# googlegenomics/spark-examples

Measured on NVIDIA H100. Metric: genotype-cells/sec (N x V) into Gram, higher is better.
Workload: dtype int8

## Files before the change

spark_examples_b200/csrc/gram_sm90.cu:

```cuda
#include <cuda.h>
#include <cuda_runtime.h>

#include <cstring>

#include <algorithm>
#include <map>
#include <mutex>
#include <tuple>
#include <type_traits>
#include <cstdio>
#include <cstdlib>
#include <string>
#include <vector>

#include "ptx_sm90.cuh"
#include "vpca_internal.h"

namespace vpca {

namespace {

constexpr int kThreads = 384;
constexpr int kKBytes = 128;
constexpr int kBoxRows = 128;
// ... 331 lines not shown
        const int cnt = kbw < kb_end - base ? kbw : kb_end - base;
        s.kb0 = base + (plan.lo[i] < cnt ? plan.lo[i] : cnt);
        s.kb1 = base + (plan.hi[i] < cnt ? plan.hi[i] : cnt);
        s.win = win;
        s.last_in_win = (seg_i == plan.n);
        s.col = plan.col[i];
        s.slot = i;
        s.first = (win == 0);
        s.flush = (win == nwin - 1);
        s.use = 0;
        return true;
    }
};

__device__ __forceinline__ void mbar_wait(uint32_t bar, uint32_t parity, int* err, int code) {
    if (ptx::mbar_try_wait(bar, parity)) return;
    const long long t0 = clock64();
    while (!ptx::mbar_try_wait(bar, parity)) {
        if (clock64() - t0 > kWatchdogCycles) {
            if (err != nullptr) {
                err[0] = code;
                err[1] = (int)blockIdx.x;
                err[2] = (int)bar;
                err[3] = (int)parity;
                __threadfence_system();
            }
            __trap();
        }
    }
}

__device__ __forceinline__ long long globaltimer_ns() {
    long long t;
    asm volatile("mov.u64 %0, %%globaltimer;" : "=l"(t));
    return t;
}

__device__ __forceinline__ void wait_window(const int* win_done, int w, int need) {
    const long long t0 = globaltimer_ns();
    while (true) {
        int v;
        asm volatile("ld.acquire.gpu.global.s32 %0, [%1];" : "=r"(v) : "l"(win_done + w) : "memory");
        if (v >= need) return;
        if (globaltimer_ns() - t0 > 200000) return;
        __nanosleep(256);
    }
}

__device__ __forceinline__ uint64_t make_smem_desc(uint32_t saddr) {
    return (uint64_t)((saddr & 0x3FFFFu) >> 4) | (1ull << 16) | ((uint64_t)(1024 >> 4) << 32) | (1ull << 62);
}

__device__ __forceinline__ uint32_t e2m1x4_to_s8x2(uint32_t w) {
    const uint32_t mag = __byte_perm(0x03020100u, 0x0C080604u, w & 0x7777u);
    const uint32_t sgn = ((w >> 3) & 1u) | (((w >> 7) & 1u) << 8) | (((w >> 11) & 1u) << 16) | (((w >> 15) & 1u) << 24);
    const uint32_t m = sgn * 0xFFu;
    return (mag & ~m) | (__vneg4(mag) & m);
}

__device__ __forceinline__ int quarter_rn(int acc) {
    const int q = acc >> 2, r = acc & 3;
    return q + ((r > 2 || (r == 2 && (q & 1))) ? 1 : 0);
}

template <int KIND>
using AccT = typename std::conditional<KIND == 1, float, uint32_t>::type;

template <int KIND>
__device__ __forceinline__ int acc_to_int(AccT<KIND> v) {
    if constexpr (KIND == 0) return (int)v;
    else if constexpr (KIND == 1) return __float2int_rn(v);
    else return quarter_rn((int)v);
}

template <int CG, int KIND>
__global__ void __launch_bounds__(kThreads, 1) gram_kernel(const __grid_constant__ CUtensorMap tmap, const GramArgs a) {
    using C = Cfg<KIND>;
    extern __shared__ uint8_t smem_raw[];
    const uint32_t smem_base = (ptx::smem_u32(smem_raw) + 1023u) & ~1023u;
    const uint32_t bar_base = smem_base + C::STAGES * C::STAGE_BYTES + C::XBUF_BYTES * 2;
    auto sB = [&](uint32_t st) { return smem_base + st * C::STAGE_BYTES; };
    auto sA = [&](uint32_t st) { return smem_base + st * C::STAGE_BYTES + C::B_BYTES; };
    auto full_bar = [&](uint32_t i) { return bar_base + 8u * i; };
    auto empty_bar = [&](uint32_t i) { return bar_base + 8u * (C::STAGES + i); };

    const int warp = __shfl_sync(0xffffffffu, (int)(threadIdx.x >> 5), 0);
    const uint32_t lane = ptx::lane_id();
    const uint32_t cta_rank = (CG == 2) ? (blockIdx.x & 1u) : 0u;
    const int worker = (CG == 2) ? (int)(blockIdx.x >> 1) : (int)blockIdx.x;
    auto release = [&](uint32_t st) {
        if constexpr (CG == 2) {
            ptx::mbar_arrive_cluster(ptx::mapa(empty_bar(st), 0));
            ptx::mbar_arrive_cluster(ptx::mapa(empty_bar(st), 1));
        } else {
            ptx::mbar_arrive(empty_bar(st));
        }
    };

    if (warp == 0 && ptx::elect_one()) {
        ptx::prefetch_tensormap(&tmap);
        for (uint32_t i = 0; i < (uint32_t)C::STAGES; ++i) {
            ptx::mbar_init(full_bar(i), 1);
            ptx::mbar_init(empty_bar(i), 2 * CG);
        }
        ptx::fence_mbar_init();
    }
    if constexpr (CG == 2) ptx::cluster_sync();
    else __syncthreads();
    if (a.prof != nullptr && threadIdx.x == 0) a.prof[(size_t)blockIdx.x * 4 + 0] = globaltimer_ns();

    if (warp < 4) {
        asm volatile("setmaxnreg.dec.sync.aligned.u32 40;");
        if (warp == 0 && ptx::elect_one()) {
            const bool leader = cta_rank == 0;
            Sched sc;
            sc.init(a, worker);
            Seg s;
            uint32_t it = 0;
            int synced_win = -1;
            while (sc.next(s)) {
                const int rowA = (CG == 2 && cta_rank != 0) ? s.rowA1 : s.rowA0;
                const bool two_boxes = s.n_eff > kBoxRows;
                const bool self_b = (CG == 2) && (s.flags & kTileSelfB) != 0;
                const uint32_t tx = (uint32_t)((two_boxes ? 2 : 1) + (self_b ? 0 : 1)) * C::BOX_BYTES;
                if (a.sync_lead > 0 && leader && s.win != synced_win) {
                    synced_win = s.win;
                    if (s.win >= a.sync_lead) wait_window(a.win_done, s.win - a.sync_lead, a.active_workers);
                }
                for (int kb = s.kb0; kb < s.kb1; ++kb, ++it) {
                    const uint32_t st = it % C::STAGES, ph = (it / C::STAGES) & 1u;
                    mbar_wait(empty_bar(st), ph ^ 1u, a.err, 1);
                    const int pnl = kb / a.kb_per_panel;
                    const int kc = (kb - pnl * a.kb_per_panel) * a.kc_per_kb;
                    ptx::mbar_arrive_expect_tx(full_bar(st), tx);
                    if constexpr (CG == 2) {
                        if (two_boxes || cta_rank == 0)
                            ptx::tma_load_3d_multicast(sB(st) + cta_rank * C::BOX_BYTES, &tmap, full_bar(st), kc,
                                                       s.rowB + (int)cta_rank * kBoxRows, pnl, 0x3);
                    } else {
                        ptx::tma_load_3d(sB(st), &tmap, full_bar(st), kc, s.rowB, pnl);
                        if (two_boxes) ptx::tma_load_3d(sB(st) + C::BOX_BYTES, &tmap, full_bar(st), kc, s.rowB + kBoxRows, pnl);
                    }
                    if (!self_b) ptx::tma_load_3d(sA(st), &tmap, full_bar(st), kc, rowA, pnl);
                }
                if (a.sync_lead > 0 && leader && s.last_in_win)
                    asm volatile("red.release.gpu.global.add.s32 [%0], 1;" ::"l"(a.win_done + s.win) : "memory");
            }
        }
    } else {
        asm volatile("setmaxnreg.inc.sync.aligned.u32 232;");
        const int cw = (warp >> 2) - 1;
        const int wq = warp & 3;
        const uint32_t ctid = threadIdx.x - 128;
        AccT<KIND> acc[2][64];
        Sched sc;
        sc.init(a, worker);
        Seg s;
        uint32_t it = 0;
        while (sc.next(s)) {
            const bool filler = (CG == 2) && cta_rank != 0 && (s.flags & kTileFiller) != 0;
            const bool self_b = (CG == 2) && (s.flags & kTileSelfB) != 0;
            const int mrow0 = cw * 128;
            const bool act0 = mrow0 < s.n_eff, act1 = mrow0 + 64 < s.n_eff;
            if (s.first) {
#pragma unroll
                for (int i = 0; i < 64; ++i) {
                    acc[0][i] = 0;
                    acc[1][i] = 0;
                }
            }
            const uint32_t a_off = (self_b ? cta_rank : 2u) * (uint32_t)(kBoxRows * 128);
            int pending = -1;
            for (int kb = s.kb0; kb < s.kb1; ++kb, ++it) {
                const uint32_t st = it % C::STAGES, ph = (it / C::STAGES) & 1u;
                mbar_wait(full_bar(st), ph, a.err, 3);
                uint32_t opB, opA;
                if constexpr (KIND == 2) {
                    const uint32_t xb = smem_base + C::STAGES * C::STAGE_BYTES + (it & 1u) * C::XBUF_BYTES;
                    ptx::named_sync(1, 256);
                    const int nb = s.n_eff > kBoxRows ? 2 * kBoxRows : kBoxRows;
                    const int rows = nb + (self_b ? 0 : kBoxRows);
                    for (int c = (int)ctid; c < rows * 8; c += 256) {
                        const int r = c >> 3, j = c & 7;
                        const uint32_t src = (r < nb ? sB(st) + (uint32_t)r * 64u : sA(st) + (uint32_t)(r - nb) * 64u) + (uint32_t)j * 8u;
                        const int xr = r < nb ? r : 2 * kBoxRows + (r - nb);
                        uint32_t lo, hi;
                        asm volatile("ld.shared.v2.u32 {%0, %1}, [%2];" : "=r"(lo), "=r"(hi) : "r"(src));
                        const uint32_t o0 = e2m1x4_to_s8x2(lo & 0xFFFFu), o1 = e2m1x4_to_s8x2(lo >> 16);
                        const uint32_t o2 = e2m1x4_to_s8x2(hi & 0xFFFFu), o3 = e2m1x4_to_s8x2(hi >> 16);
                        const uint32_t dst = xb + (uint32_t)xr * 128u + (((uint32_t)j ^ ((uint32_t)xr & 7u)) << 4);
                        asm volatile("st.shared.v4.u32 [%0], {%1, %2, %3, %4};" ::"r"(dst), "r"(o0), "r"(o1), "r"(o2), "r"(o3)
                                     : "memory");
                    }
                    ptx::fence_proxy_async();
                    ptx::named_sync(1, 256);
                    if (threadIdx.x % 128 == 0) release(st);
                    opB = xb;
                } else {
                    opB = sB(st);
                }
                opA = opB + a_off;
                const uint64_t bdesc = make_smem_desc(opA);
                const uint64_t adesc0 = make_smem_desc(opB + (uint32_t)mrow0 * 128u);
                const uint64_t adesc1 = make_smem_desc(opB + (uint32_t)(mrow0 + 64) * 128u);
                ptx::wgmma_fence_acc(acc[0]);
                ptx::wgmma_fence_acc(acc[1]);
                ptx::wgmma_fence();
#pragma unroll
                for (int k = 0; k < kKBytes / 32; ++k) {
                    if constexpr (KIND == 1) {
                        ptx::wgmma_bf16(acc[0], adesc0 + 2 * k, bdesc + 2 * k);
                        ptx::wgmma_bf16(acc[1], adesc1 + 2 * k, bdesc + 2 * k);
                    } else {
                        ptx::wgmma_s8(acc[0], adesc0 + 2 * k, bdesc + 2 * k);
                        ptx::wgmma_s8(acc[1], adesc1 + 2 * k, bdesc + 2 * k);
                    }
                }
                ptx::wgmma_commit();
                ptx::wgmma_wait<1>();
                ptx::wgmma_fence_acc(acc[0]);
                ptx::wgmma_fence_acc(acc[1]);
                if constexpr (KIND != 2) {
                    if (pending >= 0 && threadIdx.x % 128 == 0) release((uint32_t)pending);
                }
                pending = (int)st;
            }
            ptx::wgmma_wait<0>();
            ptx::wgmma_fence_acc(acc[0]);
            ptx::wgmma_fence_acc(acc[1]);
            if constexpr (KIND != 2) {
                if (pending >= 0 && threadIdx.x % 128 == 0) release((uint32_t)pending);
            }
            if (!s.flush || filler) continue;

            const int colA = (CG == 2 && cta_rank != 0) ? s.rowA1 : s.rowA0;
            const int row_end = min(a.row_limit, s.rowB + s.n_eff);
            const bool pair64 = a.red64 != 0 && (a.n & 1) == 0;
#pragma unroll
            for (int j = 0; j < 2; ++j) {
                if (!(j == 0 ? act0 : act1)) continue;
#pragma unroll
                for (int h = 0; h < 2; ++h) {
                    const int row = s.rowB + mrow0 + 64 * j + 16 * wq + (int)(lane >> 2) + 8 * h;
                    if (row >= row_end) continue;
                    int32_t* own = a.S;
                    if (a.num_peers != 0 && a.peer_mode == 1) {
                        int o = 0;
                        while (o + 1 < a.num_peers && row >= a.own_end[o]) ++o;
                        own = a.peer[o];
                    }
#pragma unroll
                    for (int i = 0; i < 16; ++i) {
                        const int col = colA + 8 * i + 2 * (int)(lane & 3);
                        if (col >= a.n) continue;
                        int v0 = acc_to_int<KIND>(acc[j][4 * i + 2 * h]);
                        int v1 = acc_to_int<KIND>(acc[j][4 * i + 2 * h + 1]);
                        if ((s.flags & kTileXpose) != 0 && (row >> 7) < (col >> 7)) {
                            for (int e = 0; e < 2; ++e) {
                                const int v = e ? v1 : v0, c = col + e;
                                if (v == 0 || c >= a.n) continue;
                                const size_t o = (size_t)c * (size_t)a.n + (size_t)row;
                                if (a.num_peers == 0) {
                                    asm volatile("red.global.add.s32 [%0], %1;" ::"l"(a.S + o), "r"(v) : "memory");
                                } else if (a.peer_mode == 1) {
                                    int q = 0;
                                    while (q + 1 < a.num_peers && c >= a.own_end[q]) ++q;
                                    asm volatile("red.relaxed.sys.global.add.s32 [%0], %1;" ::"l"(a.peer[q] + o), "r"(v) : "memory");
                                } else {
                                    for (int d = 0; d < a.num_peers; ++d)
                                        asm volatile("red.relaxed.sys.global.add.s32 [%0], %1;" ::"l"(a.peer[d] + o), "r"(v)
                                                     : "memory");
                                }
                            }
                            continue;
                        }
                        if (row < col) v0 = 0;
                        if (row < col + 1 || col + 1 >= a.n) v1 = 0;
                        if ((v0 | v1) == 0) continue;
                        const size_t o = (size_t)row * (size_t)a.n + (size_t)col;
                        if (pair64) {
                            const unsigned long long packed = (unsigned long long)(unsigned)v0 | ((unsigned long long)(unsigned)v1 << 32);
                            if (a.num_peers == 0) {
                                asm volatile("red.global.add.u64 [%0], %1;" ::"l"(a.S + o), "l"(packed) : "memory");
                            } else if (a.peer_mode == 1) {
                                asm volatile("red.relaxed.sys.global.add.u64 [%0], %1;" ::"l"(own + o), "l"(packed) : "memory");
                            } else {
                                for (int d = 0; d < a.num_peers; ++d)
                                    asm volatile("red.relaxed.sys.global.add.u64 [%0], %1;" ::"l"(a.peer[d] + o), "l"(packed)
                                                 : "memory");
                            }
                        } else {
                            for (int e = 0; e < 2; ++e) {
                                const int v = e ? v1 : v0;
                                if (v == 0) continue;
                                if (a.num_peers == 0) {
                                    asm volatile("red.global.add.s32 [%0], %1;" ::"l"(a.S + o + e), "r"(v) : "memory");
                                } else if (a.peer_mode == 1) {
                                    asm volatile("red.relaxed.sys.global.add.s32 [%0], %1;" ::"l"(own + o + e), "r"(v) : "memory");
                                } else {
                                    for (int d = 0; d < a.num_peers; ++d)
                                        asm volatile("red.relaxed.sys.global.add.s32 [%0], %1;" ::"l"(a.peer[d] + o + e), "r"(v)
                                                     : "memory");
                                }
                            }
                        }
                    }
                }
            }
        }
        if (a.prof != nullptr && threadIdx.x == 128) a.prof[(size_t)blockIdx.x * 4 + 2] = globaltimer_ns();
    }

    if constexpr (CG == 2) ptx::cluster_sync();
    else __syncthreads();
    if (a.prof != nullptr && threadIdx.x == 0) a.prof[(size_t)blockIdx.x * 4 + 3] = globaltimer_ns();
}

__global__ void rebalance_kernel(const long long* __restrict__ prof, double* __restrict__ cum, int workers, int cta_group,
                                 double gain, double max_share, long long min_ns, int* __restrict__ gen, const TileDesc* __restrict__ tiles,
                                 int num_tiles, int total_weight, int kbw, int col_limit) {
    __shared__ double sh[1024];
    __shared__ double cand[1025];
    __shared__ long long need[1025];
    __shared__ double red_sum, red_min;
    __shared__ int reject, need_repair;
    const int w = threadIdx.x;
    const bool active = w < workers;
    double t = 0.0, share_old = 0.0;
    if (active) {
        const long long t0 = prof[(size_t)w * cta_group * 4 + 0], t1 = prof[(size_t)w * cta_group * 4 + 2];
        t = (double)(t1 - t0);
        share_old = cum[w + 1] - cum[w];
    }
    sh[w] = active ? t : 1e30;
    if (w == 0) {
        reject = 0;
        need_repair = 0;
    }
    __syncthreads();
    if (w == 0) {
        double mn = 1e30, mx = 0.0;
        for (int i = 0; i < workers; ++i) {
            mn = fmin(mn, sh[i]);
            mx = fmax(mx, sh[i]);
        }
        red_min = (mn < (double)min_ns || (mx - mn) < 0.03 * mx) ? -1.0 : mn;
    }
    __syncthreads();
    if (red_min < 0.0) return;
    const double speed = active ? share_old / t : 0.0;
    sh[w] = speed;
    __syncthreads();
    if (w == 0) {
        double sum = 0.0;
        for (int i = 0; i < workers; ++i) sum += sh[i];
        red_sum = sum;
    }
    __syncthreads();
    double share = 0.0;
    if (active) {
        const double est = speed / red_sum;
        share = (1.0 - gain) * share_old + gain * est;
        const double avg = 1.0 / workers;
        share = fmin(fmax(share, 0.5 * avg), max_share * avg);
    }
    __syncthreads();
    sh[w] = share;
    __syncthreads();
    if (w == 0) {
        double sum = 0.0;
        for (int i = 0; i < workers; ++i) sum += sh[i];
        double acc = 0.0;
        cand[0] = 0.0;
        for (int i = 0; i < workers; ++i) {
            acc += sh[i] / sum;
            cand[i + 1] = (i + 1 == workers) ? 1.0 : acc;
        }
    }
    __syncthreads();
    if (active) {
        const long long uw = (long long)total_weight * kbw;
        const long long ub = (long long)((double)uw * cand[w]);
        const long long ue = (w + 1 == workers) ? uw : (long long)((double)uw * cand[w + 1]);
        int hint = 0;
        if (feasible_end(tiles, num_tiles, ub, ue, kbw, col_limit, hint) < ue) atomicExch(&need_repair, 1);
    }
    __syncthreads();
    if (need_repair && w == 0 && !repair_split(tiles, num_tiles, workers, (long long)total_weight * kbw, kbw, col_limit, cand, need)) reject = 1;
    __syncthreads();
    if (reject) return;
    if (w <= workers) cum[w] = cand[w];
    if (w == 0) *gen += 1;
}

__global__ void rebalance_front_kernel(const long long* __restrict__ prof, double* __restrict__ frac, int front, int workers,
                                       int cta_group, int kb_total, double gain, double lo, double hi, long long min_ns,
                                       int* __restrict__ gen) {
    __shared__ long long tmax[2][32];
    const int w = threadIdx.x;
    long long t = 0;
    if (w < workers) t = prof[(size_t)w * cta_group * 4 + 2] - prof[(size_t)w * cta_group * 4 + 0];
    const int side = w < front ? 0 : 1;
    long long m0 = side == 0 ? t : 0, m1 = side == 1 ? t : 0;
    for (int o = 16; o > 0; o >>= 1) {
        m0 = max(m0, __shfl_xor_sync(0xffffffffu, m0, o));
        m1 = max(m1, __shfl_xor_sync(0xffffffffu, m1, o));
    }
    if ((w & 31) == 0) {
        tmax[0][w >> 5] = m0;
        tmax[1][w >> 5] = m1;
    }
    __syncthreads();
    if (w != 0) return;
    long long tf = 0, tt = 0;
    for (int i = 0; i < (int)(blockDim.x >> 5); ++i) {
        tf = max(tf, tmax[0][i]);
        tt = max(tt, tmax[1][i]);
    }
    const double f = *frac;
    const int s = front_split(f, kb_total);
    if (s <= 0 || s >= kb_total) return;
    if (tf < min_ns || tt < min_ns) return;
    if (llabs(tf - tt) < (max(tf, tt) >> 8)) return;
    const double a = (double)tf / (double)s, b = (double)tt / (double)(kb_total - s);
    const double target = b / (a + b);
    const double nf = fmin(fmax((1.0 - gain) * f + gain * target, lo), hi);
    *frac = nf;
    *gen += 1;
}

__global__ void symmetrize_kernel(int32_t* __restrict__ S, int n) {
    __shared__ int32_t tile[32][33];
    const int bx = blockIdx.x, by = blockIdx.y;
    if (bx < by) return;
    const int tx = threadIdx.x, ty = threadIdx.y;
    for (int r = ty; r < 32; r += 8) {
        const int row = bx * 32 + r, col = by * 32 + tx;
        tile[r][tx] = (row < n && col < n) ? S[(size_t)row * n + col] : 0;
    }
    __syncthreads();
    for (int r = ty; r < 32; r += 8) {
        const int row = by * 32 + r, col = bx * 32 + tx;
        if (row < n && col < n && row < col) S[(size_t)row * n + col] = tile[tx][r];
    }
}

__global__ void add_i32_kernel(int32_t* __restrict__ dst, const int32_t* __restrict__ src, int64_t count) {
    int64_t i = (int64_t)blockIdx.x * blockDim.x + threadIdx.x;
    const int64_t stride = (int64_t)gridDim.x * blockDim.x;
    for (; i < count; i += stride) dst[i] += src[i];
}

struct PeerPtrs {
    int32_t* p[kMaxPeers];
};

// ... 757 lines not shown
```

spark_examples_b200/csrc/ptx_sm90.cuh:

```cuda
#pragma once
#include <cstdint>
#include <cuda_runtime.h>

namespace vpca {
namespace ptx {

__device__ __forceinline__ uint32_t smem_u32(const void* p) {
    return static_cast<uint32_t>(__cvta_generic_to_shared(p));
}

__device__ __forceinline__ uint32_t lane_id() {
    uint32_t r;
    asm volatile("mov.u32 %0, %%laneid;" : "=r"(r));
    return r;
}

__device__ __forceinline__ bool elect_one() {
    uint32_t pred = 0;
    asm volatile(
        "{\n\t"
        ".reg .pred P;\n\t"
        "elect.sync _|P, 0xffffffff;\n\t"
        "selp.u32 %0, 1, 0, P;\n\t"
        "}\n"
        : "=r"(pred));
    return pred != 0;
}

__device__ __forceinline__ void mbar_init(uint32_t bar, uint32_t count) {
    asm volatile("mbarrier.init.shared::cta.b64 [%0], %1;" ::"r"(bar), "r"(count) : "memory");
}
__device__ __forceinline__ void fence_mbar_init() {
    asm volatile("fence.mbarrier_init.release.cluster;" ::: "memory");
}
__device__ __forceinline__ void fence_proxy_async() {
    asm volatile("fence.proxy.async.shared::cta;" ::: "memory");
}
__device__ __forceinline__ void mbar_arrive_expect_tx(uint32_t bar, uint32_t bytes) {
    asm volatile("mbarrier.arrive.expect_tx.shared::cta.b64 _, [%0], %1;" ::"r"(bar), "r"(bytes) : "memory");
}
__device__ __forceinline__ void mbar_arrive(uint32_t bar) {
    asm volatile("mbarrier.arrive.shared::cta.b64 _, [%0];" ::"r"(bar) : "memory");
}
__device__ __forceinline__ bool mbar_try_wait(uint32_t bar, uint32_t parity) {
    uint32_t ok;
    asm volatile(
        "{\n\t"
        ".reg .pred P1;\n\t"
        "mbarrier.try_wait.parity.shared::cta.b64 P1, [%1], %2;\n\t"
        "selp.u32 %0, 1, 0, P1;\n\t"
        "}\n"
        : "=r"(ok)
        : "r"(bar), "r"(parity)
        : "memory");
    return ok != 0;
}

__device__ __forceinline__ void prefetch_tensormap(const void* desc) {
    asm volatile("prefetch.tensormap [%0];" ::"l"(reinterpret_cast<uint64_t>(desc)) : "memory");
}
__device__ __forceinline__ void tma_load_3d(uint32_t smem_dst, const void* desc, uint32_t bar, int32_t c0, int32_t c1,
                                            int32_t c2) {
    asm volatile(
        "cp.async.bulk.tensor.3d.shared::cluster.global.mbarrier::complete_tx::bytes [%0], [%1, {%3, %4, %5}], [%2];"
        ::"r"(smem_dst), "l"(reinterpret_cast<uint64_t>(desc)), "r"(bar), "r"(c0), "r"(c1), "r"(c2)
        : "memory");
}
__device__ __forceinline__ void tma_load_3d_multicast(uint32_t smem_dst, const void* desc, uint32_t bar, int32_t c0,
                                                      int32_t c1, int32_t c2, uint16_t cta_mask) {
    asm volatile(
        "cp.async.bulk.tensor.3d.shared::cluster.global.mbarrier::complete_tx::bytes.multicast::cluster"
        " [%0], [%1, {%3, %4, %5}], [%2], %6;"
        ::"r"(smem_dst), "l"(reinterpret_cast<uint64_t>(desc)), "r"(bar), "r"(c0), "r"(c1), "r"(c2), "h"(cta_mask)
        : "memory");
}
__device__ __forceinline__ uint32_t mapa(uint32_t saddr, uint32_t rank) {
    uint32_t r;
    asm volatile("mapa.shared::cluster.u32 %0, %1, %2;" : "=r"(r) : "r"(saddr), "r"(rank));
    return r;
}
__device__ __forceinline__ void mbar_arrive_cluster(uint32_t cluster_bar) {
    asm volatile("mbarrier.arrive.shared::cluster.b64 _, [%0];" ::"r"(cluster_bar) : "memory");
}
__device__ __forceinline__ void cluster_sync() {
    asm volatile("barrier.cluster.arrive.release;\n\tbarrier.cluster.wait.acquire;" ::: "memory");
}
__device__ __forceinline__ void wgmma_fence() { asm volatile("wgmma.fence.sync.aligned;" ::: "memory"); }
__device__ __forceinline__ void wgmma_commit() { asm volatile("wgmma.commit_group.sync.aligned;" ::: "memory"); }
template <int N>
__device__ __forceinline__ void wgmma_wait() { asm volatile("wgmma.wait_group.sync.aligned %0;" ::"n"(N) : "memory"); }
__device__ __forceinline__ void wgmma_fence_acc(uint32_t (&d)[64]) {
#pragma unroll
    for (int i = 0; i < 64; ++i) asm volatile("" : "+r"(d[i])::"memory");
}
__device__ __forceinline__ void wgmma_fence_acc(float (&d)[64]) {
#pragma unroll
    for (int i = 0; i < 64; ++i) asm volatile("" : "+f"(d[i])::"memory");
}

__device__ __forceinline__ void wgmma_s8(uint32_t (&d)[64], uint64_t a_desc, uint64_t b_desc) {
    asm volatile(
        "{\n\t.reg .pred p;\n\tsetp.ne.b32 p, 1, 0;\n\t"
        "wgmma.mma_async.sync.aligned.m64n128k32.s32.s8.s8 "
        "{%0, %1, %2, %3, %4, %5, %6, %7, %8, %9, %10, %11, %12, %13, %14, %15, %16, %17, %18, %19, %20, %21, %22, %23, %24, %25, %26, %27, %28, %29, %30, %31, %32, %33, %34, %35, %36, %37, %38, %39, %40, %41, %42, %43, %44, %45, %46, %47, %48, %49, %50, %51, %52, %53, %54, %55, %56, %57, %58, %59, %60, %61, %62, %63}, %64, %65, p;\n\t}\n"
        : "+r"(d[0]), "+r"(d[1]), "+r"(d[2]), "+r"(d[3]), "+r"(d[4]), "+r"(d[5]), "+r"(d[6]), "+r"(d[7]), "+r"(d[8]), "+r"(d[9]), "+r"(d[10]), "+r"(d[11]), "+r"(d[12]), "+r"(d[13]), "+r"(d[14]), "+r"(d[15]), "+r"(d[16]), "+r"(d[17]), "+r"(d[18]), "+r"(d[19]), "+r"(d[20]), "+r"(d[21]), "+r"(d[22]), "+r"(d[23]), "+r"(d[24]), "+r"(d[25]), "+r"(d[26]), "+r"(d[27]), "+r"(d[28]), "+r"(d[29]), "+r"(d[30]), "+r"(d[31]), "+r"(d[32]), "+r"(d[33]), "+r"(d[34]), "+r"(d[35]), "+r"(d[36]), "+r"(d[37]), "+r"(d[38]), "+r"(d[39]), "+r"(d[40]), "+r"(d[41]), "+r"(d[42]), "+r"(d[43]), "+r"(d[44]), "+r"(d[45]), "+r"(d[46]), "+r"(d[47]), "+r"(d[48]), "+r"(d[49]), "+r"(d[50]), "+r"(d[51]), "+r"(d[52]), "+r"(d[53]), "+r"(d[54]), "+r"(d[55]), "+r"(d[56]), "+r"(d[57]), "+r"(d[58]), "+r"(d[59]), "+r"(d[60]), "+r"(d[61]), "+r"(d[62]), "+r"(d[63])
        : "l"(a_desc), "l"(b_desc));
}

__device__ __forceinline__ void wgmma_bf16(float (&f)[64], uint64_t a_desc, uint64_t b_desc) {
    asm volatile(
        "{\n\t.reg .pred p;\n\tsetp.ne.b32 p, 1, 0;\n\t"
        "wgmma.mma_async.sync.aligned.m64n128k16.f32.bf16.bf16 "
        "{%0, %1, %2, %3, %4, %5, %6, %7, %8, %9, %10, %11, %12, %13, %14, %15, %16, %17, %18, %19, %20, %21, %22, %23, %24, %25, %26, %27, %28, %29, %30, %31, %32, %33, %34, %35, %36, %37, %38, %39, %40, %41, %42, %43, %44, %45, %46, %47, %48, %49, %50, %51, %52, %53, %54, %55, %56, %57, %58, %59, %60, %61, %62, %63}, %64, %65, p, 1, 1, 0, 0;\n\t}\n"
        : "+f"(f[0]), "+f"(f[1]), "+f"(f[2]), "+f"(f[3]), "+f"(f[4]), "+f"(f[5]), "+f"(f[6]), "+f"(f[7]), "+f"(f[8]), "+f"(f[9]), "+f"(f[10]), "+f"(f[11]), "+f"(f[12]), "+f"(f[13]), "+f"(f[14]), "+f"(f[15]), "+f"(f[16]), "+f"(f[17]), "+f"(f[18]), "+f"(f[19]), "+f"(f[20]), "+f"(f[21]), "+f"(f[22]), "+f"(f[23]), "+f"(f[24]), "+f"(f[25]), "+f"(f[26]), "+f"(f[27]), "+f"(f[28]), "+f"(f[29]), "+f"(f[30]), "+f"(f[31]), "+f"(f[32]), "+f"(f[33]), "+f"(f[34]), "+f"(f[35]), "+f"(f[36]), "+f"(f[37]), "+f"(f[38]), "+f"(f[39]), "+f"(f[40]), "+f"(f[41]), "+f"(f[42]), "+f"(f[43]), "+f"(f[44]), "+f"(f[45]), "+f"(f[46]), "+f"(f[47]), "+f"(f[48]), "+f"(f[49]), "+f"(f[50]), "+f"(f[51]), "+f"(f[52]), "+f"(f[53]), "+f"(f[54]), "+f"(f[55]), "+f"(f[56]), "+f"(f[57]), "+f"(f[58]), "+f"(f[59]), "+f"(f[60]), "+f"(f[61]), "+f"(f[62]), "+f"(f[63])
        : "l"(a_desc), "l"(b_desc));
}

__device__ __forceinline__ void named_sync(uint32_t id, uint32_t count) {
    asm volatile("bar.sync %0, %1;" ::"r"(id), "r"(count) : "memory");
}

}
}
```

Baseline: 627.4 billion.

## Switch consumer WGMMA to m64n256 tiles with swapped operands and shuffled epilogue

Each consumer warpgroup now issues one m64n256 WGMMA per k-step instead of two m64n128 ones. The operands are swapped so the 256-wide B tile spans the row block and each warpgroup owns 64 columns of the A tile. When the effective row count fits in one box, an n128 variant is selected through a compile-time lambda specialization. The epilogue is rewritten for the transposed accumulator layout, using a warp shuffle to pair adjacent columns so that packed 64-bit reductions still work. The intent is to halve WGMMA issue count and descriptor overhead and improve B-operand reuse per instruction. In exchange the epilogue gains shuffles, and register pressure and the tile mapping change.

Result: faster. 641.7 billion, median of 6 (+2.3%).

```diff
diff --git a/spark_examples_b200/csrc/gram_sm90.cu b/spark_examples_b200/csrc/gram_sm90.cu
--- a/spark_examples_b200/csrc/gram_sm90.cu
+++ b/spark_examples_b200/csrc/gram_sm90.cu
@@ -507,7 +507,7 @@
         const int cw = (warp >> 2) - 1;
         const int wq = warp & 3;
         const uint32_t ctid = threadIdx.x - 128;
-        AccT<KIND> acc[2][64];
+        AccT<KIND> acc[128];
         Sched sc;
         sc.init(a, worker);
         Seg s;
@@ -515,74 +515,71 @@
         while (sc.next(s)) {
             const bool filler = (CG == 2) && cta_rank != 0 && (s.flags & kTileFiller) != 0;
             const bool self_b = (CG == 2) && (s.flags & kTileSelfB) != 0;
-            const int mrow0 = cw * 128;
-            const bool act0 = mrow0 < s.n_eff, act1 = mrow0 + 64 < s.n_eff;
+            const bool n128 = s.n_eff <= kBoxRows;
             if (s.first) {
 #pragma unroll
-                for (int i = 0; i < 64; ++i) {
-                    acc[0][i] = 0;
-                    acc[1][i] = 0;
+                for (int i = 0; i < 128; ++i) acc[i] = 0;
+            }
+            const uint32_t a_off = (self_b ? cta_rank : 2u) * (uint32_t)(kBoxRows * 128) + (uint32_t)cw * 64u * 128u;
+            int pending = -1;
+            auto kblocks = [&](auto n_const) {
+                constexpr int N = decltype(n_const)::value;
+                for (int kb = s.kb0; kb < s.kb1; ++kb, ++it) {
+                    const uint32_t st = it % C::STAGES, ph = (it / C::STAGES) & 1u;
+                    mbar_wait(full_bar(st), ph, a.err, 3);
+                    uint32_t opB, opA;
+                    if constexpr (KIND == 2) {
+                        const uint32_t xb = smem_base + C::STAGES * C::STAGE_BYTES + (it & 1u) * C::XBUF_BYTES;
+                        ptx::named_sync(1, 256);
+                        const int nb = s.n_eff > kBoxRows ? 2 * kBoxRows : kBoxRows;
+                        const int rows = nb + (self_b ? 0 : kBoxRows);
+                        for (int c = (int)ctid; c < rows * 8; c += 256) {
+                            const int r = c >> 3, j = c & 7;
+                            const uint32_t src = (r < nb ? sB(st) + (uint32_t)r * 64u : sA(st) + (uint32_t)(r - nb) * 64u) + (uint32_t)j * 8u;
+                            const int xr = r < nb ? r : 2 * kBoxRows + (r - nb);
+                            uint32_t lo, hi;
+                            asm volatile("ld.shared.v2.u32 {%0, %1}, [%2];" : "=r"(lo), "=r"(hi) : "r"(src));
+                            const uint32_t o0 = e2m1x4_to_s8x2(lo & 0xFFFFu), o1 = e2m1x4_to_s8x2(lo >> 16);
+                            const uint32_t o2 = e2m1x4_to_s8x2(hi & 0xFFFFu), o3 = e2m1x4_to_s8x2(hi >> 16);
+                            const uint32_t dst = xb + (uint32_t)xr * 128u + (((uint32_t)j ^ ((uint32_t)xr & 7u)) << 4);
+                            asm volatile("st.shared.v4.u32 [%0], {%1, %2, %3, %4};" ::"r"(dst), "r"(o0), "r"(o1), "r"(o2), "r"(o3)
+                                         : "memory");
+                        }
+                        ptx::fence_proxy_async();
+                        ptx::named_sync(1, 256);
+                        if (threadIdx.x % 128 == 0) release(st);
+                        opB = xb;
+                    } else {
+                        opB = sB(st);
+                    }
+                    opA = opB + a_off;
+                    const uint64_t adesc = make_smem_desc(opA);
+                    const uint64_t bdesc = make_smem_desc(opB);
+                    ptx::wgmma_fence_acc(acc);
+                    ptx::wgmma_fence();
+#pragma unroll
+                    for (int k = 0; k < kKBytes / 32; ++k) {
+                        if constexpr (N == 256) {
+                            if constexpr (KIND == 1) ptx::wgmma_bf16_n256(acc, adesc + 2 * k, bdesc + 2 * k);
+                            else ptx::wgmma_s8_n256(acc, adesc + 2 * k, bdesc + 2 * k);
+                        } else {
+                            if constexpr (KIND == 1) ptx::wgmma_bf16_n128(acc, adesc + 2 * k, bdesc + 2 * k);
+                            else ptx::wgmma_s8_n128(acc, adesc + 2 * k, bdesc + 2 * k);
+                        }
+                    }
+                    ptx::wgmma_commit();
+                    ptx::wgmma_wait<1>();
+                    ptx::wgmma_fence_acc(acc);
+                    if constexpr (KIND != 2) {
+                        if (pending >= 0 && threadIdx.x % 128 == 0) release((uint32_t)pending);
+                    }
+                    pending = (int)st;
                 }
-            }
-            const uint32_t a_off = (self_b ? cta_rank : 2u) * (uint32_t)(kBoxRows * 128);
-            int pending = -1;
-            for (int kb = s.kb0; kb < s.kb1; ++kb, ++it) {
-                const uint32_t st = it % C::STAGES, ph = (it / C::STAGES) & 1u;
-                mbar_wait(full_bar(st), ph, a.err, 3);
-                uint32_t opB, opA;
-                if constexpr (KIND == 2) {
-                    const uint32_t xb = smem_base + C::STAGES * C::STAGE_BYTES + (it & 1u) * C::XBUF_BYTES;
-                    ptx::named_sync(1, 256);
-                    const int nb = s.n_eff > kBoxRows ? 2 * kBoxRows : kBoxRows;
-                    const int rows = nb + (self_b ? 0 : kBoxRows);
-                    for (int c = (int)ctid; c < rows * 8; c += 256) {
-                        const int r = c >> 3, j = c & 7;
-                        const uint32_t src = (r < nb ? sB(st) + (uint32_t)r * 64u : sA(st) + (uint32_t)(r - nb) * 64u) + (uint32_t)j * 8u;
-                        const int xr = r < nb ? r : 2 * kBoxRows + (r - nb);
-                        uint32_t lo, hi;
-                        asm volatile("ld.shared.v2.u32 {%0, %1}, [%2];" : "=r"(lo), "=r"(hi) : "r"(src));
-                        const uint32_t o0 = e2m1x4_to_s8x2(lo & 0xFFFFu), o1 = e2m1x4_to_s8x2(lo >> 16);
-                        const uint32_t o2 = e2m1x4_to_s8x2(hi & 0xFFFFu), o3 = e2m1x4_to_s8x2(hi >> 16);
-                        const uint32_t dst = xb + (uint32_t)xr * 128u + (((uint32_t)j ^ ((uint32_t)xr & 7u)) << 4);
-                        asm volatile("st.shared.v4.u32 [%0], {%1, %2, %3, %4};" ::"r"(dst), "r"(o0), "r"(o1), "r"(o2), "r"(o3)
-                                     : "memory");
-                    }
-                    ptx::fence_proxy_async();
-                    ptx::named_sync(1, 256);
-                    if (threadIdx.x % 128 == 0) release(st);
-                    opB = xb;
-                } else {
-                    opB = sB(st);
-                }
-                opA = opB + a_off;
-                const uint64_t bdesc = make_smem_desc(opA);
-                const uint64_t adesc0 = make_smem_desc(opB + (uint32_t)mrow0 * 128u);
-                const uint64_t adesc1 = make_smem_desc(opB + (uint32_t)(mrow0 + 64) * 128u);
-                ptx::wgmma_fence_acc(acc[0]);
-                ptx::wgmma_fence_acc(acc[1]);
-                ptx::wgmma_fence();
-#pragma unroll
-                for (int k = 0; k < kKBytes / 32; ++k) {
-                    if constexpr (KIND == 1) {
-                        ptx::wgmma_bf16(acc[0], adesc0 + 2 * k, bdesc + 2 * k);
-                        ptx::wgmma_bf16(acc[1], adesc1 + 2 * k, bdesc + 2 * k);
-                    } else {
-                        ptx::wgmma_s8(acc[0], adesc0 + 2 * k, bdesc + 2 * k);
-                        ptx::wgmma_s8(acc[1], adesc1 + 2 * k, bdesc + 2 * k);
-                    }
-                }
-                ptx::wgmma_commit();
-                ptx::wgmma_wait<1>();
-                ptx::wgmma_fence_acc(acc[0]);
-                ptx::wgmma_fence_acc(acc[1]);
-                if constexpr (KIND != 2) {
-                    if (pending >= 0 && threadIdx.x % 128 == 0) release((uint32_t)pending);
-                }
-                pending = (int)st;
-            }
+            };
+            if (n128) kblocks(std::integral_constant<int, 128>{});
+            else kblocks(std::integral_constant<int, 256>{});
             ptx::wgmma_wait<0>();
-            ptx::wgmma_fence_acc(acc[0]);
-            ptx::wgmma_fence_acc(acc[1]);
+            ptx::wgmma_fence_acc(acc);
             if constexpr (KIND != 2) {
                 if (pending >= 0 && threadIdx.x % 128 == 0) release((uint32_t)pending);
             }
@@ -591,72 +588,79 @@
             const int colA = (CG == 2 && cta_rank != 0) ? s.rowA1 : s.rowA0;
             const int row_end = min(a.row_limit, s.rowB + s.n_eff);
             const bool pair64 = a.red64 != 0 && (a.n & 1) == 0;
+            const uint32_t odd = (lane >> 2) & 1u;
+            const int col_w = colA + 64 * cw + 16 * wq + (int)((lane >> 2) & ~1u);
 #pragma unroll
-            for (int j = 0; j < 2; ++j) {
-                if (!(j == 0 ? act0 : act1)) continue;
+            for (int i = 0; i < 32; ++i) {
+                if (n128 && i >= 16) break;
+                const int row = s.rowB + 8 * i + 2 * (int)(lane & 3) + (int)odd;
+                AccT<KIND> p0[2], p1[2];
 #pragma unroll
                 for (int h = 0; h < 2; ++h) {
-                    const int row = s.rowB + mrow0 + 64 * j + 16 * wq + (int)(lane >> 2) + 8 * h;
-                    if (row >= row_end) continue;
-                    int32_t* own = a.S;
-                    if (a.num_peers != 0 && a.peer_mode == 1) {
-                        int o = 0;
-                        while (o + 1 < a.num_peers && row >= a.own_end[o]) ++o;
-                        own = a.peer[o];
-                    }
+                    const AccT<KIND> x0 = acc[4 * i + 2 * h], x1 = acc[4 * i + 2 * h + 1];
+                    const AccT<KIND> got = __shfl_xor_sync(0xffffffffu, odd ? x0 : x1, 4);
+                    p0[h] = odd ? got : x0;
+                    p1[h] = odd ? x1 : got;
+                }
+                if (row >= row_end) continue;
+                int32_t* own = a.S;
+                if (a.num_peers != 0 && a.peer_mode == 1) {
+                    int o = 0;
+                    while (o + 1 < a.num_peers && row >= a.own_end[o]) ++o;
+                    own = a.peer[o];
+                }
 #pragma unroll
-                    for (int i = 0; i < 16; ++i) {
-                        const int col = colA + 8 * i + 2 * (int)(lane & 3);
-                        if (col >= a.n) continue;
-                        int v0 = acc_to_int<KIND>(acc[j][4 * i + 2 * h]);
-                        int v1 = acc_to_int<KIND>(acc[j][4 * i + 2 * h + 1]);
-                        if ((s.flags & kTileXpose) != 0 && (row >> 7) < (col >> 7)) {
-                            for (int e = 0; e < 2; ++e) {
-                                const int v = e ? v1 : v0, c = col + e;
-                                if (v == 0 || c >= a.n) continue;
-                                const size_t o = (size_t)c * (size_t)a.n + (size_t)row;
-                                if (a.num_peers == 0) {
-                                    asm volatile("red.global.add.s32 [%0], %1;" ::"l"(a.S + o), "r"(v) : "memory");
-                                } else if (a.peer_mode == 1) {
-                                    int q = 0;
-                                    while (q + 1 < a.num_peers && c >= a.own_end[q]) ++q;
-                                    asm volatile("red.relaxed.sys.global.add.s32 [%0], %1;" ::"l"(a.peer[q] + o), "r"(v) : "memory");
-                                } else {
-                                    for (int d = 0; d < a.num_peers; ++d)
-                                        asm volatile("red.relaxed.sys.global.add.s32 [%0], %1;" ::"l"(a.peer[d] + o), "r"(v)
-                                                     : "memory");
-                                }
-                            }
-                            continue;
-                        }
-                        if (row < col) v0 = 0;
-                        if (row < col + 1 || col + 1 >= a.n) v1 = 0;
-                        if ((v0 | v1) == 0) continue;
-                        const size_t o = (size_t)row * (size_t)a.n + (size_t)col;
-                        if (pair64) {
-                            const unsigned long long packed = (unsigned long long)(unsigned)v0 | ((unsigned long long)(unsigned)v1 << 32);
+                for (int h = 0; h < 2; ++h) {
+                    const int col = col_w + 8 * h;
+                    if (col >= a.n) continue;
+                    int v0 = acc_to_int<KIND>(p0[h]);
+                    int v1 = acc_to_int<KIND>(p1[h]);
+                    if ((s.flags & kTileXpose) != 0 && (row >> 7) < (col >> 7)) {
+                        for (int e = 0; e < 2; ++e) {
+                            const int v = e ? v1 : v0, c = col + e;
+                            if (v == 0 || c >= a.n) continue;
+                            const size_t o = (size_t)c * (size_t)a.n + (size_t)row;
                             if (a.num_peers == 0) {
-                                asm volatile("red.global.add.u64 [%0], %1;" ::"l"(a.S + o), "l"(packed) : "memory");
+                                asm volatile("red.global.add.s32 [%0], %1;" ::"l"(a.S + o), "r"(v) : "memory");
                             } else if (a.peer_mode == 1) {
-                                asm volatile("red.relaxed.sys.global.add.u64 [%0], %1;" ::"l"(own + o), "l"(packed) : "memory");
+                                int q = 0;
+                                while (q + 1 < a.num_peers && c >= a.own_end[q]) ++q;
+                                asm volatile("red.relaxed.sys.global.add.s32 [%0], %1;" ::"l"(a.peer[q] + o), "r"(v) : "memory");
                             } else {
                                 for (int d = 0; d < a.num_peers; ++d)
-                                    asm volatile("red.relaxed.sys.global.add.u64 [%0], %1;" ::"l"(a.peer[d] + o), "l"(packed)
+                                    asm volatile("red.relaxed.sys.global.add.s32 [%0], %1;" ::"l"(a.peer[d] + o), "r"(v)
                                                  : "memory");
                             }
+                        }
+                        continue;
+                    }
+                    if (row < col) v0 = 0;
+                    if (row < col + 1 || col + 1 >= a.n) v1 = 0;
+                    if ((v0 | v1) == 0) continue;
+                    const size_t o = (size_t)row * (size_t)a.n + (size_t)col;
+                    if (pair64) {
+                        const unsigned long long packed = (unsigned long long)(unsigned)v0 | ((unsigned long long)(unsigned)v1 << 32);
+                        if (a.num_peers == 0) {
+                            asm volatile("red.global.add.u64 [%0], %1;" ::"l"(a.S + o), "l"(packed) : "memory");
+                        } else if (a.peer_mode == 1) {
+                            asm volatile("red.relaxed.sys.global.add.u64 [%0], %1;" ::"l"(own + o), "l"(packed) : "memory");
                         } else {
-                            for (int e = 0; e < 2; ++e) {
-                                const int v = e ? v1 : v0;
-                                if (v == 0) continue;
-                                if (a.num_peers == 0) {
-                                    asm volatile("red.global.add.s32 [%0], %1;" ::"l"(a.S + o + e), "r"(v) : "memory");
-                                } else if (a.peer_mode == 1) {
-                                    asm volatile("red.relaxed.sys.global.add.s32 [%0], %1;" ::"l"(own + o + e), "r"(v) : "memory");
-                                } else {
-                                    for (int d = 0; d < a.num_peers; ++d)
-                                        asm volatile("red.relaxed.sys.global.add.s32 [%0], %1;" ::"l"(a.peer[d] + o + e), "r"(v)
-                                                     : "memory");
-                                }
+                            for (int d = 0; d < a.num_peers; ++d)
+                                asm volatile("red.relaxed.sys.global.add.u64 [%0], %1;" ::"l"(a.peer[d] + o), "l"(packed)
+                                             : "memory");
+                        }
+                    } else {
+                        for (int e = 0; e < 2; ++e) {
+                            const int v = e ? v1 : v0;
+                            if (v == 0) continue;
+                            if (a.num_peers == 0) {
+                                asm volatile("red.global.add.s32 [%0], %1;" ::"l"(a.S + o + e), "r"(v) : "memory");
+                            } else if (a.peer_mode == 1) {
+                                asm volatile("red.relaxed.sys.global.add.s32 [%0], %1;" ::"l"(own + o + e), "r"(v) : "memory");
+                            } else {
+                                for (int d = 0; d < a.num_peers; ++d)
+                                    asm volatile("red.relaxed.sys.global.add.s32 [%0], %1;" ::"l"(a.peer[d] + o + e), "r"(v)
+                                                 : "memory");
                             }
                         }
                     }
diff --git a/spark_examples_b200/csrc/ptx_sm90.cuh b/spark_examples_b200/csrc/ptx_sm90.cuh
--- a/spark_examples_b200/csrc/ptx_sm90.cuh
+++ b/spark_examples_b200/csrc/ptx_sm90.cuh
@@ -89,16 +89,16 @@
 __device__ __forceinline__ void wgmma_commit() { asm volatile("wgmma.commit_group.sync.aligned;" ::: "memory"); }
 template <int N>
 __device__ __forceinline__ void wgmma_wait() { asm volatile("wgmma.wait_group.sync.aligned %0;" ::"n"(N) : "memory"); }
-__device__ __forceinline__ void wgmma_fence_acc(uint32_t (&d)[64]) {
+__device__ __forceinline__ void wgmma_fence_acc(uint32_t (&d)[128]) {
 #pragma unroll
-    for (int i = 0; i < 64; ++i) asm volatile("" : "+r"(d[i])::"memory");
+    for (int i = 0; i < 128; ++i) asm volatile("" : "+r"(d[i])::"memory");
 }
-__device__ __forceinline__ void wgmma_fence_acc(float (&d)[64]) {
+__device__ __forceinline__ void wgmma_fence_acc(float (&d)[128]) {
 #pragma unroll
-    for (int i = 0; i < 64; ++i) asm volatile("" : "+f"(d[i])::"memory");
+    for (int i = 0; i < 128; ++i) asm volatile("" : "+f"(d[i])::"memory");
 }
 
-__device__ __forceinline__ void wgmma_s8(uint32_t (&d)[64], uint64_t a_desc, uint64_t b_desc) {
+__device__ __forceinline__ void wgmma_s8_n128(uint32_t (&d)[128], uint64_t a_desc, uint64_t b_desc) {
     asm volatile(
         "{\n\t.reg .pred p;\n\tsetp.ne.b32 p, 1, 0;\n\t"
         "wgmma.mma_async.sync.aligned.m64n128k32.s32.s8.s8 "
@@ -107,12 +107,30 @@
         : "l"(a_desc), "l"(b_desc));
 }
 
-__device__ __forceinline__ void wgmma_bf16(float (&f)[64], uint64_t a_desc, uint64_t b_desc) {
+__device__ __forceinline__ void wgmma_bf16_n128(float (&f)[128], uint64_t a_desc, uint64_t b_desc) {
     asm volatile(
         "{\n\t.reg .pred p;\n\tsetp.ne.b32 p, 1, 0;\n\t"
         "wgmma.mma_async.sync.aligned.m64n128k16.f32.bf16.bf16 "
         "{%0, %1, %2, %3, %4, %5, %6, %7, %8, %9, %10, %11, %12, %13, %14, %15, %16, %17, %18, %19, %20, %21, %22, %23, %24, %25, %26, %27, %28, %29, %30, %31, %32, %33, %34, %35, %36, %37, %38, %39, %40, %41, %42, %43, %44, %45, %46, %47, %48, %49, %50, %51, %52, %53, %54, %55, %56, %57, %58, %59, %60, %61, %62, %63}, %64, %65, p, 1, 1, 0, 0;\n\t}\n"
         : "+f"(f[0]), "+f"(f[1]), "+f"(f[2]), "+f"(f[3]), "+f"(f[4]), "+f"(f[5]), "+f"(f[6]), "+f"(f[7]), "+f"(f[8]), "+f"(f[9]), "+f"(f[10]), "+f"(f[11]), "+f"(f[12]), "+f"(f[13]), "+f"(f[14]), "+f"(f[15]), "+f"(f[16]), "+f"(f[17]), "+f"(f[18]), "+f"(f[19]), "+f"(f[20]), "+f"(f[21]), "+f"(f[22]), "+f"(f[23]), "+f"(f[24]), "+f"(f[25]), "+f"(f[26]), "+f"(f[27]), "+f"(f[28]), "+f"(f[29]), "+f"(f[30]), "+f"(f[31]), "+f"(f[32]), "+f"(f[33]), "+f"(f[34]), "+f"(f[35]), "+f"(f[36]), "+f"(f[37]), "+f"(f[38]), "+f"(f[39]), "+f"(f[40]), "+f"(f[41]), "+f"(f[42]), "+f"(f[43]), "+f"(f[44]), "+f"(f[45]), "+f"(f[46]), "+f"(f[47]), "+f"(f[48]), "+f"(f[49]), "+f"(f[50]), "+f"(f[51]), "+f"(f[52]), "+f"(f[53]), "+f"(f[54]), "+f"(f[55]), "+f"(f[56]), "+f"(f[57]), "+f"(f[58]), "+f"(f[59]), "+f"(f[60]), "+f"(f[61]), "+f"(f[62]), "+f"(f[63])
+        : "l"(a_desc), "l"(b_desc));
+}
+
+__device__ __forceinline__ void wgmma_s8_n256(uint32_t (&d)[128], uint64_t a_desc, uint64_t b_desc) {
+    asm volatile(
+        "{\n\t.reg .pred p;\n\tsetp.ne.b32 p, 1, 0;\n\t"
+        "wgmma.mma_async.sync.aligned.m64n256k32.s32.s8.s8 "
+        "{%0, %1, %2, %3, %4, %5, %6, %7, %8, %9, %10, %11, %12, %13, %14, %15, %16, %17, %18, %19, %20, %21, %22, %23, %24, %25, %26, %27, %28, %29, %30, %31, %32, %33, %34, %35, %36, %37, %38, %39, %40, %41, %42, %43, %44, %45, %46, %47, %48, %49, %50, %51, %52, %53, %54, %55, %56, %57, %58, %59, %60, %61, %62, %63, %64, %65, %66, %67, %68, %69, %70, %71, %72, %73, %74, %75, %76, %77, %78, %79, %80, %81, %82, %83, %84, %85, %86, %87, %88, %89, %90, %91, %92, %93, %94, %95, %96, %97, %98, %99, %100, %101, %102, %103, %104, %105, %106, %107, %108, %109, %110, %111, %112, %113, %114, %115, %116, %117, %118, %119, %120, %121, %122, %123, %124, %125, %126, %127}, %128, %129, p;\n\t}\n"
+        : "+r"(d[0]), "+r"(d[1]), "+r"(d[2]), "+r"(d[3]), "+r"(d[4]), "+r"(d[5]), "+r"(d[6]), "+r"(d[7]), "+r"(d[8]), "+r"(d[9]), "+r"(d[10]), "+r"(d[11]), "+r"(d[12]), "+r"(d[13]), "+r"(d[14]), "+r"(d[15]), "+r"(d[16]), "+r"(d[17]), "+r"(d[18]), "+r"(d[19]), "+r"(d[20]), "+r"(d[21]), "+r"(d[22]), "+r"(d[23]), "+r"(d[24]), "+r"(d[25]), "+r"(d[26]), "+r"(d[27]), "+r"(d[28]), "+r"(d[29]), "+r"(d[30]), "+r"(d[31]), "+r"(d[32]), "+r"(d[33]), "+r"(d[34]), "+r"(d[35]), "+r"(d[36]), "+r"(d[37]), "+r"(d[38]), "+r"(d[39]), "+r"(d[40]), "+r"(d[41]), "+r"(d[42]), "+r"(d[43]), "+r"(d[44]), "+r"(d[45]), "+r"(d[46]), "+r"(d[47]), "+r"(d[48]), "+r"(d[49]), "+r"(d[50]), "+r"(d[51]), "+r"(d[52]), "+r"(d[53]), "+r"(d[54]), "+r"(d[55]), "+r"(d[56]), "+r"(d[57]), "+r"(d[58]), "+r"(d[59]), "+r"(d[60]), "+r"(d[61]), "+r"(d[62]), "+r"(d[63]), "+r"(d[64]), "+r"(d[65]), "+r"(d[66]), "+r"(d[67]), "+r"(d[68]), "+r"(d[69]), "+r"(d[70]), "+r"(d[71]), "+r"(d[72]), "+r"(d[73]), "+r"(d[74]), "+r"(d[75]), "+r"(d[76]), "+r"(d[77]), "+r"(d[78]), "+r"(d[79]), "+r"(d[80]), "+r"(d[81]), "+r"(d[82]), "+r"(d[83]), "+r"(d[84]), "+r"(d[85]), "+r"(d[86]), "+r"(d[87]), "+r"(d[88]), "+r"(d[89]), "+r"(d[90]), "+r"(d[91]), "+r"(d[92]), "+r"(d[93]), "+r"(d[94]), "+r"(d[95]), "+r"(d[96]), "+r"(d[97]), "+r"(d[98]), "+r"(d[99]), "+r"(d[100]), "+r"(d[101]), "+r"(d[102]), "+r"(d[103]), "+r"(d[104]), "+r"(d[105]), "+r"(d[106]), "+r"(d[107]), "+r"(d[108]), "+r"(d[109]), "+r"(d[110]), "+r"(d[111]), "+r"(d[112]), "+r"(d[113]), "+r"(d[114]), "+r"(d[115]), "+r"(d[116]), "+r"(d[117]), "+r"(d[118]), "+r"(d[119]), "+r"(d[120]), "+r"(d[121]), "+r"(d[122]), "+r"(d[123]), "+r"(d[124]), "+r"(d[125]), "+r"(d[126]), "+r"(d[127])
+        : "l"(a_desc), "l"(b_desc));
+}
+
+__device__ __forceinline__ void wgmma_bf16_n256(float (&d)[128], uint64_t a_desc, uint64_t b_desc) {
+    asm volatile(
+        "{\n\t.reg .pred p;\n\tsetp.ne.b32 p, 1, 0;\n\t"
+        "wgmma.mma_async.sync.aligned.m64n256k16.f32.bf16.bf16 "
+        "{%0, %1, %2, %3, %4, %5, %6, %7, %8, %9, %10, %11, %12, %13, %14, %15, %16, %17, %18, %19, %20, %21, %22, %23, %24, %25, %26, %27, %28, %29, %30, %31, %32, %33, %34, %35, %36, %37, %38, %39, %40, %41, %42, %43, %44, %45, %46, %47, %48, %49, %50, %51, %52, %53, %54, %55, %56, %57, %58, %59, %60, %61, %62, %63, %64, %65, %66, %67, %68, %69, %70, %71, %72, %73, %74, %75, %76, %77, %78, %79, %80, %81, %82, %83, %84, %85, %86, %87, %88, %89, %90, %91, %92, %93, %94, %95, %96, %97, %98, %99, %100, %101, %102, %103, %104, %105, %106, %107, %108, %109, %110, %111, %112, %113, %114, %115, %116, %117, %118, %119, %120, %121, %122, %123, %124, %125, %126, %127}, %128, %129, p, 1, 1, 0, 0;\n\t}\n"
+        : "+f"(d[0]), "+f"(d[1]), "+f"(d[2]), "+f"(d[3]), "+f"(d[4]), "+f"(d[5]), "+f"(d[6]), "+f"(d[7]), "+f"(d[8]), "+f"(d[9]), "+f"(d[10]), "+f"(d[11]), "+f"(d[12]), "+f"(d[13]), "+f"(d[14]), "+f"(d[15]), "+f"(d[16]), "+f"(d[17]), "+f"(d[18]), "+f"(d[19]), "+f"(d[20]), "+f"(d[21]), "+f"(d[22]), "+f"(d[23]), "+f"(d[24]), "+f"(d[25]), "+f"(d[26]), "+f"(d[27]), "+f"(d[28]), "+f"(d[29]), "+f"(d[30]), "+f"(d[31]), "+f"(d[32]), "+f"(d[33]), "+f"(d[34]), "+f"(d[35]), "+f"(d[36]), "+f"(d[37]), "+f"(d[38]), "+f"(d[39]), "+f"(d[40]), "+f"(d[41]), "+f"(d[42]), "+f"(d[43]), "+f"(d[44]), "+f"(d[45]), "+f"(d[46]), "+f"(d[47]), "+f"(d[48]), "+f"(d[49]), "+f"(d[50]), "+f"(d[51]), "+f"(d[52]), "+f"(d[53]), "+f"(d[54]), "+f"(d[55]), "+f"(d[56]), "+f"(d[57]), "+f"(d[58]), "+f"(d[59]), "+f"(d[60]), "+f"(d[61]), "+f"(d[62]), "+f"(d[63]), "+f"(d[64]), "+f"(d[65]), "+f"(d[66]), "+f"(d[67]), "+f"(d[68]), "+f"(d[69]), "+f"(d[70]), "+f"(d[71]), "+f"(d[72]), "+f"(d[73]), "+f"(d[74]), "+f"(d[75]), "+f"(d[76]), "+f"(d[77]), "+f"(d[78]), "+f"(d[79]), "+f"(d[80]), "+f"(d[81]), "+f"(d[82]), "+f"(d[83]), "+f"(d[84]), "+f"(d[85]), "+f"(d[86]), "+f"(d[87]), "+f"(d[88]), "+f"(d[89]), "+f"(d[90]), "+f"(d[91]), "+f"(d[92]), "+f"(d[93]), "+f"(d[94]), "+f"(d[95]), "+f"(d[96]), "+f"(d[97]), "+f"(d[98]), "+f"(d[99]), "+f"(d[100]), "+f"(d[101]), "+f"(d[102]), "+f"(d[103]), "+f"(d[104]), "+f"(d[105]), "+f"(d[106]), "+f"(d[107]), "+f"(d[108]), "+f"(d[109]), "+f"(d[110]), "+f"(d[111]), "+f"(d[112]), "+f"(d[113]), "+f"(d[114]), "+f"(d[115]), "+f"(d[116]), "+f"(d[117]), "+f"(d[118]), "+f"(d[119]), "+f"(d[120]), "+f"(d[121]), "+f"(d[122]), "+f"(d[123]), "+f"(d[124]), "+f"(d[125]), "+f"(d[126]), "+f"(d[127])
         : "l"(a_desc), "l"(b_desc));
 }
 
```
